# vision-agh/apse_uav

Measured on AMD Instinct MI355X. Metric: 4K UAV frames/sec (whole node), higher is better.
Workload: dtype f32

## Files before the change

### apse_uav_amd/csrc/conv_winograd.hip

```cpp
#include "apse_common.h"

namespace {
constexpr int WTR = 16, WTC = 4;
constexpr int WT = WTR * WTC;
constexpr int WN = 64;
constexpr int KC = 8;
constexpr int NTHR = 512;
constexpr int G_U = 1, G_ROWS = 2, G_V = 3;
constexpr int SLICE_F = 16 * WT * KC;
constexpr size_t WINO_LDS = (size_t)2 * 2 * SLICE_F * sizeof(float);
static_assert(WN == WT, "V and U slices share one size");
static_assert((size_t)16 * WT * 32 * sizeof(float) <= WINO_LDS, "epilogue chunk must fit the staging LDS");
}

__global__ __launch_bounds__(NTHR) void conv_winograd_f32(const ConvParams p) {
    extern __shared__ __attribute__((aligned(16))) char smem[];
    float* Vs = reinterpret_cast<float*>(smem);
    float* Us = Vs + 2 * SLICE_F;
    float* Cs = reinterpret_cast<float*>(smem);

    const int tid = threadIdx.x;
    const int lane = tid & 63, wave = __builtin_amdgcn_readfirstlane(tid >> 6);
    const int fr = lane & 31, fh = lane >> 5;

    const int tiles_y = (p.OH + 2 * WTR - 1) / (2 * WTR), tiles_x = (p.OW + 2 * WTC - 1) / (2 * WTC);
    const int nblk = p.Cout / WN;
    const int nwg = p.B * tiles_y * tiles_x * nblk;
    int bid;
    {
        const int wg = blockIdx.x;
        const int q = nwg >> 3, r = nwg & 7, xcd = wg & 7, idx = wg >> 3;
        bid = (xcd < r ? xcd * (q + 1) : r * (q + 1) + (xcd - r) * q) + idx;
    }
    const int nb = bid % nblk;
    int rest = bid / nblk;
    const int bx = rest % tiles_x; rest /= tiles_x;
    const int by = rest % tiles_y;
    const int b = rest / tiles_y;
    const int oy0 = by * 2 * WTR, ox0 = bx * 2 * WTC, n0 = nb * WN;
    const int C = 1 << p.cin_log2;
    const int nsteps = C / KC;

    const int cg = tid & 1, t = (tid >> 1) & (WT - 1), ti = wave >> 1;
    const int ra = ti == 0 ? 0 : (ti == 2 ? 2 : 1);
    const int rb = ti == 0 ? 2 : (ti == 1 ? 2 : (ti == 2 ? 1 : 3));
    const float sgn = ti == 1 ? 1.f : -1.f;
    const int iy_a = oy0 + 2 * (t / WTC) - 1 + ra, iy_b = oy0 + 2 * (t / WTC) - 1 + rb;
    const int ix0 = ox0 + 2 * (t % WTC) - 1;
    const __amdgpu_buffer_rsrc_t xrsrc =
        __builtin_amdgcn_make_buffer_rsrc(const_cast<float*>(p.x), 0, (int)((((unsigned)(p.B * p.H * p.W)) << p.cin_log2) * 4u), 0x00020000);
    const __amdgpu_buffer_rsrc_t xnone = __builtin_amdgcn_make_buffer_rsrc(const_cast<float*>(p.x), 0, 0, 0x00020000);
    unsigned xoff[2][4];
#pragma unroll
    for (int r = 0; r < 2; ++r) {
        const int iy = r ? iy_b : iy_a;
#pragma unroll
        for (int c = 0; c < 4; ++c) {
            const int ix = ix0 + c;
            const bool in = (unsigned)iy < (unsigned)p.H && (unsigned)ix < (unsigned)p.W;
            xoff[r][c] = in ? ((((unsigned)((b * p.H + iy) * p.W + ix)) << p.cin_log2) + (unsigned)(cg * 4)) * 4u : 0x80000000u;
        }
    }
    const __amdgpu_buffer_rsrc_t ursrc =
        __builtin_amdgcn_make_buffer_rsrc(const_cast<float*>(p.wu), 0, (int)((((unsigned)(16 * p.Cout)) << p.cin_log2) * 4u), 0x00020000);
    const unsigned ustep = (unsigned)(16 * p.Cout * KC * 4);
    unsigned uoff[4], ulds[4];
#pragma unroll
    for (int k = 0; k < 4; ++k) {
        const int q = tid + NTHR * k;
        const int xi = q >> 7, co = (q >> 1) & 63, h = q & 1;
        uoff[k] = (unsigned)(((xi * p.Cout + n0 + co) * KC + h * 4) * 4);
        ulds[k] = (unsigned)((xi * WN + co) * KC + ((h ^ ((co >> 3) & 1)) * 4));
    }
    const int vlds = (4 * ti * WT + t) * KC + (cg ^ ((t >> 3) & 1)) * 4;

    f32x4 xr[2][4], ur[4];
    auto fetch_u = [&](int s) {
        const unsigned kb = (unsigned)s * ustep;
#pragma unroll
        for (int k = 0; k < 4; ++k) ur[k] = __builtin_bit_cast(f32x4, __builtin_amdgcn_raw_buffer_load_b128(ursrc, (int)(uoff[k] + kb), 0, 0));
    };
    auto fetch_x = [&](int s) {
        const unsigned kb = (unsigned)(s * KC * 4);
        const __amdgpu_buffer_rsrc_t rs = s < nsteps ? xrsrc : xnone;
#pragma unroll
        for (int r = 0; r < 2; ++r)
#pragma unroll
            for (int c = 0; c < 4; ++c)
                xr[r][c] = __builtin_bit_cast(f32x4, __builtin_amdgcn_raw_buffer_load_b128(rs, (int)(xoff[r][c] + kb), 0, 0));
    };
    auto write_u = [&](int buf) {
#pragma unroll
        for (int k = 0; k < 4; ++k) *reinterpret_cast<f32x4*>(Us + buf * SLICE_F + ulds[k]) = ur[k];
    };
    auto xform_rows = [&]() {
#pragma unroll
        for (int c = 0; c < 4; ++c)
#pragma unroll
            for (int e = 0; e < 4; ++e) xr[0][c][e] = __builtin_fmaf(xr[1][c][e], sgn, xr[0][c][e]);
    };
    auto write_v = [&](int buf) {
        const f32x4 v[4] = {xr[0][0] - xr[0][2], xr[0][1] + xr[0][2], xr[0][2] - xr[0][1], xr[0][1] - xr[0][3]};
#pragma unroll
        for (int j = 0; j < 4; ++j) *reinterpret_cast<f32x4*>(Vs + buf * SLICE_F + vlds + j * WT * KC) = v[j];
    };

    f32x16 acc[2][2][2];
#pragma unroll
    for (int a = 0; a < 2; ++a)
#pragma unroll
        for (int i = 0; i < 2; ++i)
#pragma unroll
            for (int j = 0; j < 2; ++j)
#pragma unroll
                for (int v = 0; v < 16; ++v) acc[a][i][j][v] = 0.f;

    fetch_u(0);
    fetch_x(0);
    write_u(0);
    xform_rows();
    write_v(0);
    __builtin_amdgcn_sched_barrier(0);
    fetch_u(1);
    __builtin_amdgcn_sched_barrier(0);
    fetch_x(1);
    __syncthreads();
    const int fsw = (fh ^ ((fr >> 3) & 1)) * 4;
    const int frag = (2 * wave * WT + fr) * KC + fsw;
    f32x4 af[2][2], bf[2][2];
    auto read_frags = [&](int buf, int a) {
#pragma unroll
        for (int i = 0; i < 2; ++i) af[a][i] = *reinterpret_cast<const f32x4*>(Vs + buf * SLICE_F + frag + (a * WT + 32 * i) * KC);
#pragma unroll
        for (int j = 0; j < 2; ++j) bf[a][j] = *reinterpret_cast<const f32x4*>(Us + buf * SLICE_F + frag + (a * WN + 32 * j) * KC);
    };
    auto mfma_group = [&](int a, int k) {
#pragma unroll
        for (int i = 0; i < 2; ++i)
#pragma unroll
            for (int j = 0; j < 2; ++j)
                acc[a][i][j] = __builtin_amdgcn_mfma_f32_32x32x2f32(af[a][i][k], bf[a][j][k], acc[a][i][j], 0, 0, 0);
    };
    read_frags(0, 0);
    for (int s = 0; s < nsteps; ++s) {
        const int buf = s & 1;
        read_frags(buf, 1);
#pragma unroll
        for (int g = 0; g < 7; ++g) {
            __builtin_amdgcn_sched_barrier(0);
            if (g == G_U) { write_u(buf ^ 1); fetch_u(s + 2); }
            if (g == G_ROWS) xform_rows();
            if (g == G_V) { write_v(buf ^ 1); fetch_x(s + 2); }
            __builtin_amdgcn_sched_barrier(0);
            mfma_group(g >> 2, g & 3);
        }
        __builtin_amdgcn_sched_barrier(0);
        __syncthreads();
        read_frags(buf ^ 1, 0);
        __builtin_amdgcn_sched_barrier(0);
        mfma_group(1, 3);
    }

    const int et = tid >> 3, eg = tid & 7;
    const int oy = oy0 + 2 * (et / WTC), ox = ox0 + 2 * (et % WTC);
    typedef unsigned u32x4_t __attribute__((ext_vector_type(4)));
#pragma unroll
    for (int j = 0; j < 2; ++j) {
#pragma unroll
        for (int a = 0; a < 2; ++a)
#pragma unroll
            for (int i = 0; i < 2; ++i)
#pragma unroll
                for (int v = 0; v < 16; ++v) {
                    const int row = 32 * i + (v & 3) + 8 * (v >> 2) + 4 * fh;
                    Cs[((2 * wave + a) * WT + row) * 32 + fr] = acc[a][i][j][v];
                }
        __syncthreads();
        f32x4 m[16];
#pragma unroll
        for (int k = 0; k < 16; ++k) m[k] = *reinterpret_cast<const f32x4*>(Cs + (k * WT + et) * 32 + eg * 4);
        f32x4 s0[4], s1[4];
#pragma unroll
        for (int c = 0; c < 4; ++c) {
            s0[c] = m[c] + m[4 + c] + m[8 + c];
            s1[c] = m[4 + c] - m[8 + c] - m[12 + c];
        }
        const int co = n0 + 32 * j + 4 * eg;
        const f32x4 bias4 = p.bias ? *reinterpret_cast<const f32x4*>(p.bias + co) : f32x4{0.f, 0.f, 0.f, 0.f};
        f32x4 y[2][2] = {{s0[0] + s0[1] + s0[2], s0[1] - s0[2] - s0[3]}, {s1[0] + s1[1] + s1[2], s1[1] - s1[2] - s1[3]}};
#pragma unroll
        for (int dy = 0; dy < 2; ++dy)
#pragma unroll
            for (int dx = 0; dx < 2; ++dx) {
                f32x4 val = y[dy][dx] + bias4;
                if (p.relu) {
#pragma unroll
                    for (int k = 0; k < 4; ++k) val[k] = apse_relu(val[k]);
                }
                if (oy + dy < p.OH && ox + dx < p.OW)
                    APSE_NT_STORE(val, reinterpret_cast<f32x4*>(p.y + ((size_t)(b * p.OH + oy + dy) * p.OW + ox + dx) * p.y_ld + p.y_coff + co));
            }
        __syncthreads();
    }
}

bool apse_conv_winograd_ok(const ConvParams& p, int max_items) {
    return p.prec == 0 && p.x_st == 0 && p.y_st == 0 && p.KH == 3 && p.KW == 3 && p.stride == 1 && p.pad == 1 && p.out_mode == 0 &&
           p.res_mode == 0 && p.splitk == 1 && p.Cout % WN == 0 && p.cin_log2 >= 3 && p.OH == p.H && p.OW == p.W &&
           (p.y_ld & 3) == 0 && (p.y_coff & 3) == 0 && ((((size_t)max_items * p.H * p.W) << p.cin_log2) * 4 < 0x7fff0000ull);
}

int apse_conv_winograd_blocks(const ConvParams& p) {
    return ((p.OH + 2 * WTR - 1) / (2 * WTR)) * ((p.OW + 2 * WTC - 1) / (2 * WTC)) * (p.Cout / WN);
}

int apse_launch_conv_winograd(const ConvParams& p, hipStream_t s, hipEvent_t ev0, hipEvent_t ev1) {
    if (!p.wu || !apse_conv_winograd_ok(p, p.B) || p.m_count) return APSE_E_INVALID;
    static bool attr_done = false;
    if (!attr_done) {
        hipFuncSetAttribute(reinterpret_cast<const void*>(&conv_winograd_f32), hipFuncAttributeMaxDynamicSharedMemorySize, (int)WINO_LDS);
        attr_done = true;
    }
    const int tiles_y = (p.OH + 2 * WTR - 1) / (2 * WTR), tiles_x = (p.OW + 2 * WTC - 1) / (2 * WTC);
    const int grid = p.B * tiles_y * tiles_x * (p.Cout / WN);
    if (ev0) hipEventRecord(ev0, s);
    hipLaunchKernelGGL(conv_winograd_f32, dim3(grid), dim3(NTHR), WINO_LDS, s, p);
    if (ev1) hipEventRecord(ev1, s);
    return hipGetLastError() == hipSuccess ? APSE_OK : APSE_E_HIP;
}
```

Measured before the change: 194.9.

## Stage input patch in LDS and DMA weight slices directly into LDS

Result: no change. 195.8, median of 6 (+0.5%).

```diff
diff --git a/apse_uav_amd/csrc/conv_winograd.hip b/apse_uav_amd/csrc/conv_winograd.hip
--- a/apse_uav_amd/csrc/conv_winograd.hip
+++ b/apse_uav_amd/csrc/conv_winograd.hip
@@ -1,4 +1,10 @@
 #include "apse_common.h"
+
+#ifndef WG_ABLATE
+#define WG_ABLATE 0
+#endif
+
+typedef __attribute__((address_space(3))) void* wg_lds_ptr_t;
 
 namespace {
 constexpr int WTR = 16, WTC = 4;
@@ -6,9 +12,15 @@
 constexpr int WN = 64;
 constexpr int KC = 8;
 constexpr int NTHR = 512;
-constexpr int G_U = 1, G_ROWS = 2, G_V = 3;
+constexpr int G_ROWS = 2, G_V = 3;
+constexpr int G_DMA = 0, G_TAPS = 0, G_P = 5;
 constexpr int SLICE_F = 16 * WT * KC;
-constexpr size_t WINO_LDS = (size_t)2 * 2 * SLICE_F * sizeof(float);
+constexpr int PROWS = 2 * WTR + 2, PCOLS = 2 * WTC + 2;
+constexpr int NPIECE = PROWS * PCOLS * 2;
+constexpr int PPITCH = 84;
+constexpr int PATCH_F = PROWS * PPITCH;
+static_assert(NPIECE > NTHR && NPIECE <= 2 * NTHR, "two pieces per thread");
+constexpr size_t WINO_LDS = (size_t)(2 * 2 * SLICE_F + 2 * PATCH_F) * sizeof(float);
 static_assert(WN == WT, "V and U slices share one size");
 static_assert((size_t)16 * WT * 32 * sizeof(float) <= WINO_LDS, "epilogue chunk must fit the staging LDS");
 }
@@ -17,6 +29,7 @@
     extern __shared__ __attribute__((aligned(16))) char smem[];
     float* Vs = reinterpret_cast<float*>(smem);
     float* Us = Vs + 2 * SLICE_F;
+    float* Ps = Us + 2 * SLICE_F;
     float* Cs = reinterpret_cast<float*>(smem);
 
     const int tid = threadIdx.x;
@@ -45,53 +58,59 @@
     const int ra = ti == 0 ? 0 : (ti == 2 ? 2 : 1);
     const int rb = ti == 0 ? 2 : (ti == 1 ? 2 : (ti == 2 ? 1 : 3));
     const float sgn = ti == 1 ? 1.f : -1.f;
-    const int iy_a = oy0 + 2 * (t / WTC) - 1 + ra, iy_b = oy0 + 2 * (t / WTC) - 1 + rb;
-    const int ix0 = ox0 + 2 * (t % WTC) - 1;
     const __amdgpu_buffer_rsrc_t xrsrc =
         __builtin_amdgcn_make_buffer_rsrc(const_cast<float*>(p.x), 0, (int)((((unsigned)(p.B * p.H * p.W)) << p.cin_log2) * 4u), 0x00020000);
     const __amdgpu_buffer_rsrc_t xnone = __builtin_amdgcn_make_buffer_rsrc(const_cast<float*>(p.x), 0, 0, 0x00020000);
-    unsigned xoff[2][4];
-#pragma unroll
-    for (int r = 0; r < 2; ++r) {
-        const int iy = r ? iy_b : iy_a;
-#pragma unroll
-        for (int c = 0; c < 4; ++c) {
-            const int ix = ix0 + c;
-            const bool in = (unsigned)iy < (unsigned)p.H && (unsigned)ix < (unsigned)p.W;
-            xoff[r][c] = in ? ((((unsigned)((b * p.H + iy) * p.W + ix)) << p.cin_log2) + (unsigned)(cg * 4)) * 4u : 0x80000000u;
-        }
-    }
+    unsigned poff[2];
+    int plds[2];
+#pragma unroll
+    for (int k = 0; k < 2; ++k) {
+        const int q = (tid + NTHR * k) % NPIECE;
+        const int pix = q >> 1, h = q & 1, pr = pix / PCOLS, pc = pix - pr * PCOLS;
+        const int iy = oy0 - 1 + pr, ix = ox0 - 1 + pc;
+        const bool in = (unsigned)iy < (unsigned)p.H && (unsigned)ix < (unsigned)p.W;
+        poff[k] = in ? ((((unsigned)((b * p.H + iy) * p.W + ix)) << p.cin_log2) + (unsigned)(h * 4)) * 4u : 0x80000000u;
+        plds[k] = pr * PPITCH + pc * KC + h * 4;
+    }
+    const int tap_a = (2 * (t / WTC) + ra) * PPITCH + 2 * (t % WTC) * KC + cg * 4;
+    const int tap_b = (2 * (t / WTC) + rb) * PPITCH + 2 * (t % WTC) * KC + cg * 4;
     const __amdgpu_buffer_rsrc_t ursrc =
         __builtin_amdgcn_make_buffer_rsrc(const_cast<float*>(p.wu), 0, (int)((((unsigned)(16 * p.Cout)) << p.cin_log2) * 4u), 0x00020000);
+    const __amdgpu_buffer_rsrc_t ufrom = (WG_ABLATE & 2) ? xnone : ursrc;
     const unsigned ustep = (unsigned)(16 * p.Cout * KC * 4);
-    unsigned uoff[4], ulds[4];
+    unsigned uoff[4];
 #pragma unroll
     for (int k = 0; k < 4; ++k) {
         const int q = tid + NTHR * k;
         const int xi = q >> 7, co = (q >> 1) & 63, h = q & 1;
-        uoff[k] = (unsigned)(((xi * p.Cout + n0 + co) * KC + h * 4) * 4);
-        ulds[k] = (unsigned)((xi * WN + co) * KC + ((h ^ ((co >> 3) & 1)) * 4));
-    }
+        uoff[k] = (unsigned)(((xi * p.Cout + n0 + co) * KC + (h ^ ((co >> 3) & 1)) * 4) * 4);
+    }
+    auto dma_u = [&](int s, int buf) {
+        const unsigned kb = (unsigned)s * ustep;
+#pragma unroll
+        for (int k = 0; k < 4; ++k)
+            __builtin_amdgcn_raw_ptr_buffer_load_lds(ufrom, (wg_lds_ptr_t)(smem + (size_t)(2 * SLICE_F + buf * SLICE_F + (NTHR * k + 64 * wave) * 4) * sizeof(float)), 16,
+                                                     (int)(uoff[k] + kb), 0, 0, 0);
+    };
     const int vlds = (4 * ti * WT + t) * KC + (cg ^ ((t >> 3) & 1)) * 4;
 
-    f32x4 xr[2][4], ur[4];
-    auto fetch_u = [&](int s) {
-        const unsigned kb = (unsigned)s * ustep;
-#pragma unroll
-        for (int k = 0; k < 4; ++k) ur[k] = __builtin_bit_cast(f32x4, __builtin_amdgcn_raw_buffer_load_b128(ursrc, (int)(uoff[k] + kb), 0, 0));
-    };
-    auto fetch_x = [&](int s) {
+    f32x4 xr[2][4], pr[2];
+    auto fetch_p = [&](int s) {
         const unsigned kb = (unsigned)(s * KC * 4);
-        const __amdgpu_buffer_rsrc_t rs = s < nsteps ? xrsrc : xnone;
-#pragma unroll
-        for (int r = 0; r < 2; ++r)
-#pragma unroll
-            for (int c = 0; c < 4; ++c)
-                xr[r][c] = __builtin_bit_cast(f32x4, __builtin_amdgcn_raw_buffer_load_b128(rs, (int)(xoff[r][c] + kb), 0, 0));
-    };
-    auto write_u = [&](int buf) {
-#pragma unroll
-        for (int k = 0; k < 4; ++k) *reinterpret_cast<f32x4*>(Us + buf * SLICE_F + ulds[k]) = ur[k];
+        const __amdgpu_buffer_rsrc_t rs = (s < nsteps && !(WG_ABLATE & 1)) ? xrsrc : xnone;
+#pragma unroll
+        for (int k = 0; k < 2; ++k) pr[k] = __builtin_bit_cast(f32x4, __builtin_amdgcn_raw_buffer_load_b128(rs, (int)(poff[k] + kb), 0, 0));
+    };
+    auto write_p = [&](int pb) {
+#pragma unroll
+        for (int k = 0; k < 2; ++k) *reinterpret_cast<f32x4*>(Ps + pb * PATCH_F + plds[k]) = pr[k];
+    };
+    auto read_taps = [&](int pb) {
+#pragma unroll
+        for (int c = 0; c < 4; ++c) {
+            xr[0][c] = *reinterpret_cast<const f32x4*>(Ps + pb * PATCH_F + tap_a + c * KC);
+            xr[1][c] = *reinterpret_cast<const f32x4*>(Ps + pb * PATCH_F + tap_b + c * KC);
+        }
     };
     auto xform_rows = [&]() {
 #pragma unroll
@@ -115,15 +134,18 @@
 #pragma unroll
                 for (int v = 0; v < 16; ++v) acc[a][i][j][v] = 0.f;
 
-    fetch_u(0);
-    fetch_x(0);
-    write_u(0);
+    dma_u(0, 0);
+    fetch_p(0);
+    write_p(0);
+    fetch_p(1);
+    __syncthreads();
+    read_taps(0);
     xform_rows();
     write_v(0);
+    write_p(1);
     __builtin_amdgcn_sched_barrier(0);
-    fetch_u(1);
-    __builtin_amdgcn_sched_barrier(0);
-    fetch_x(1);
+    fetch_p(2);
+    asm volatile("s_waitcnt vmcnt(2)" ::: "memory");
     __syncthreads();
     const int fsw = (fh ^ ((fr >> 3) & 1)) * 4;
     const int frag = (2 * wave * WT + fr) * KC + fsw;
@@ -148,13 +170,16 @@
 #pragma unroll
         for (int g = 0; g < 7; ++g) {
             __builtin_amdgcn_sched_barrier(0);
-            if (g == G_U) { write_u(buf ^ 1); fetch_u(s + 2); }
+            if (g == G_DMA) dma_u(s + 1, buf ^ 1);
+            if (g == G_TAPS) read_taps(buf ^ 1);
             if (g == G_ROWS) xform_rows();
-            if (g == G_V) { write_v(buf ^ 1); fetch_x(s + 2); }
+            if (g == G_V) write_v(buf ^ 1);
+            if (g == G_P) { write_p(buf); fetch_p(s + 3); }
             __builtin_amdgcn_sched_barrier(0);
             mfma_group(g >> 2, g & 3);
         }
         __builtin_amdgcn_sched_barrier(0);
+        asm volatile("s_waitcnt vmcnt(2)" ::: "memory");
         __syncthreads();
         read_frags(buf ^ 1, 0);
         __builtin_amdgcn_sched_barrier(0);
```
